# wilkinsdr/raytrace_cpu

Measured on AMD Instinct MI355X. Metric: rays_per_sec, higher is better.
Workload: dtype f64

## Files before the change

raytrace_cpu_amd/csrc/kr_trace.hip:

```cpp

#include <hip/hip_runtime.h>

#include <algorithm>
#include <atomic>
#include <cmath>
#include <cstdio>
#include <cstdlib>
#include <cstring>
#include <iterator>
#include <limits>
#include <map>
#include <mutex>
#include <type_traits>
#include <vector>

#include "kr_common.hpp"
#include "kr_device.hpp"
#include "kr_post_device.hpp"
#include "kr_ray_io.hpp"

namespace kr {

namespace {

constexpr int kBlock = 256;
constexpr int kTraceBlock = 64;
#ifndef KR_REFILL_MIN
#define KR_REFILL_MIN 4
#endif
constexpr int kLongRaySteps = 2048;
#ifndef KR_OCC_STATS
#define KR_OCC_STATS 0
#endif
enum CounterWord { kHead, kTraced, kSteps, kAttempts, kRejects, kStationary, kExtrapolated, kLongest, kCounterWords,
                   kFlagged = kTraced };
constexpr int kCounters = KR_OCC_STATS ? 13 : kCounterWords;
enum CounterBlock { kMainBlock, kSideBlock, kOverflowBlock, kSplitBlock, kCounterBlocks };
constexpr int kListCap = 32768;

template <typename T> struct RayOf;
template <> struct RayOf<double> { using type = kr_ray_f64; };
template <> struct RayOf<float> { using type = kr_ray_f32; };

KR_DEV unsigned long long wave_max(unsigned long long v)
{
#pragma unroll
    for (int off = 32; off > 0; off >>= 1) {
        const unsigned long long o = __shfl_down(v, off, 64);
        v = o > v ? o : v;
    }
    return v;
}

template <typename T> KR_DEV unsigned long long wave_sum(unsigned long long v)
{
#pragma unroll
    for (int off = 32; off > 0; off >>= 1) v += __shfl_down(v, off, 64);
    return v;
}

#define KR_WAVES_ATTR __attribute__((amdgpu_waves_per_eu(HOG ? 1 : METHOD == KR_RK4 ? 3 : METHOD == KR_RK45 ? 2 : 4, 8)))
template <typename T> struct TraceDesc {
    typename RayOf<T>::type* rays;
    long long n;
    TraceConsts<T> c;
    unsigned long long* counters;
    const int* list = nullptr;
    const unsigned long long* n_ptr = nullptr;
    const unsigned char* mask = nullptr;
    int n_mode = 0, mask_want = 0;
};

template <typename T, int METHOD, bool USE_DEST, bool FAST, bool HOG, int REFILL_MIN>
KR_DEV void trace_body(typename RayOf<T>::type* __restrict__ rays, long long n, const TraceConsts<T>& c, unsigned long long* __restrict__ counters,
                       const int* __restrict__ list, const unsigned long long* __restrict__ n_ptr, int n_mode, const unsigned char* __restrict__ mask, int mask_want,
                       int& has_prio, long long first_slot = -1, unsigned long long head_offset = 0)
{
    if (n_ptr) {
        const long long m = (long long) *n_ptr;
        n = (n_mode == 1) ? (m < n ? m : n) : (m > (long long) kListCap ? n : 0);
    }
    const int lane = threadIdx.x & 63;
    const unsigned long long lane_bit = 1ull << lane;

    Lane<T> s;
    long long idx = -1;
    bool have = false;
    bool pend = false;
    bool exhausted = false;
    unsigned long long my_steps = 0, my_traced = 0;
    int32_t my_longest = 0;
    uint32_t my_attempts = 0, my_rejects = 0, my_stationary = 0, my_creep = 0;

#if KR_OCC_STATS
    unsigned long long occ_iters = 0, occ_tail_iters = 0, occ_tail_steps = 0, occ_refills = 0, occ_refill_lanes = 0;
#endif
    for (;;) {
        const unsigned long long need = __builtin_amdgcn_ballot_w64(!have);
        const int n_need = __popcll(need);
        const bool any_have = (need != ~0ull);

        const bool visit = !exhausted && n_need > 0 && (n_need >= REFILL_MIN || !any_have);
        const bool leaving = !visit && !any_have;
        if (visit || leaving) {
            if (pend) {
                my_steps += (unsigned long long) s.steps;
                my_longest = s.steps > my_longest ? s.steps : my_longest;
                store_ray(&rays[idx], s, finish_status<T, USE_DEST>(s, c));
                pend = false;
            }
            if (leaving) break;
            if constexpr (!HOG) {
                const int32_t st = have ? s.steps : 0;
                auto any = [](bool x) { return __builtin_amdgcn_ballot_w64(x) != 0; };
                const int want_prio = any(st > 8 * kLongRaySteps) ? 3 : any(st > 3 * kLongRaySteps) ? 2 : any(st > kLongRaySteps) ? 1 : 0;
                if (want_prio != has_prio) {
                    has_prio = want_prio;
                    switch (want_prio) {
                        case 3: __builtin_amdgcn_s_setprio(3); break;
                        case 2: __builtin_amdgcn_s_setprio(2); break;
                        case 1: __builtin_amdgcn_s_setprio(1); break;
                        default: __builtin_amdgcn_s_setprio(0); break;
                    }
                }
            }
#if KR_OCC_STATS
            ++occ_refills; occ_refill_lanes += n_need;
#endif
            const int leader = __ffsll((long long) need) - 1;
            unsigned long long base = 0;
            if (first_slot >= 0) {
                base = (unsigned long long) first_slot;
                first_slot = -1;
            } else {
                if (lane == leader) base = atomicAdd(&counters[kHead], (unsigned long long) n_need);
                base = __shfl(base, leader, 64) + head_offset;
            }
            if (base + (unsigned long long) n_need >= (unsigned long long) n) exhausted = true;
            if (!have) {
                const long long slot = (long long) base + __popcll(need & (lane_bit - 1));
                if (slot < n) {
                    long long mine = slot;
                    if constexpr (HOG) { if (list) mine = (long long) list[slot]; }
                    const unsigned char* launch = mask ? mask + slot : (const unsigned char*) &rays[mine];
                    const unsigned char launch_of_ray = *launch;
                    load_ray(&rays[mine], s);
                    if ((!mask || launch_of_ray == (unsigned char) mask_want) && s.steps0 >= 0 && s.steps0 < c.steplim) {
                        idx = mine;
                        have = true;
                        ++my_traced;
                        s.steps = 0;
                        s.r_was_positive = false;
                        s.theta_was_positive = true;
                        s.in_retry = false;
                        s.creep_m = 0;
                        s.creep_run = 0;
                        s.creep_mode = false;
                        s.fsal_valid = false;
                        energy_guard_set(s);
                        if (METHOD == KR_RK45) rk45_seed(s, c);
                        if (!loop_cond<T, USE_DEST>(s, c)) {
                            have = false;
                            pend = true;
                        }
                    }
                }
            }
            continue;
        }

        int replay_batch = 1;
        if constexpr (METHOD == KR_RK45 && sizeof(T) == 8) {
            if (!__any(have && !s.creep_mode)) replay_batch = 16;
        }
#if KR_OCC_STATS
        ++occ_iters;
        if (exhausted) { ++occ_tail_iters; occ_tail_steps += have ? 1 : 0; }
#endif
        if (have) {
            bool fin;
            if (METHOD == KR_EULER) fin = step_fixed<T, false, USE_DEST, FAST, HOG>(s, c);
            else if (METHOD == KR_RK4) fin = step_fixed<T, true, USE_DEST, FAST, HOG>(s, c);
            else fin = step_rk45<T, USE_DEST, FAST, HOG>(s, c, my_attempts, my_rejects, my_stationary, my_creep, replay_batch);
            if (fin) {
                have = false;
                pend = true;
            }
        }
    }
    const unsigned long long w_traced = wave_sum<T>(my_traced);
    const unsigned long long w_steps = wave_sum<T>(my_steps);
    const unsigned long long w_att = wave_sum<T>((unsigned long long) my_attempts);
    const unsigned long long w_rej = wave_sum<T>((unsigned long long) my_rejects);
    const unsigned long long w_sta = wave_sum<T>((unsigned long long) my_stationary);
    const unsigned long long w_creep = wave_sum<T>((unsigned long long) my_creep);
    const unsigned long long w_longest = wave_max((unsigned long long) my_longest);
#if KR_OCC_STATS
    {
        const unsigned long long w_tail_steps = wave_sum<T>(occ_tail_steps);
        if (lane == 0) {
            atomicAdd(&counters[8], occ_iters); atomicAdd(&counters[9], occ_tail_iters); atomicAdd(&counters[10], w_tail_steps);
            atomicAdd(&counters[11], occ_refills); atomicAdd(&counters[12], occ_refill_lanes);
        }
    }
#endif
    if (lane == 0) {
        if (w_longest) atomicMax(&counters[kLongest], w_longest);
        if (w_sta) atomicAdd(&counters[kStationary], w_sta);
        if (w_creep) atomicAdd(&counters[kExtrapolated], w_creep);
        if (w_traced) atomicAdd(&counters[kTraced], w_traced);
        if (w_steps) atomicAdd(&counters[kSteps], w_steps);
        if (w_att) atomicAdd(&counters[kAttempts], w_att);
        if (w_rej) atomicAdd(&counters[kRejects], w_rej);
    }
}

template <typename T> KR_DEV void consts_into_vector_registers(TraceConsts<T>& c)
{
    if constexpr (sizeof(T) == 8) {
        auto hold = [](T& x) { asm("" : "+v"(x)); };
        hold(c.a); hold(c.horizon); hold(c.rlim); hold(c.precision); hold(c.theta_precision); hold(c.max_tstep); hold(c.tol);
        hold(c.inv_precision); hold(c.inv_theta_precision); hold(c.tstep_rlim_eff); hold(c.phistep_eff); hold(c.theta_lo); hold(c.theta_hi);
    }
}

template <typename T, int METHOD, bool USE_DEST, bool FAST, bool HOG, int REFILL_MIN>
__global__ void __attribute__((amdgpu_flat_work_group_size(kTraceBlock, kTraceBlock))) KR_WAVES_ATTR
trace_kernel(typename RayOf<T>::type* __restrict__ rays, long long n, TraceConsts<T> c, unsigned long long* __restrict__ counters,
             const int* __restrict__ list, const unsigned long long* __restrict__ n_ptr, int n_mode, const unsigned char* __restrict__ mask, int mask_want)
{
    if (HOG) asm volatile("; claim the whole register file" ::: "v255", "a255");
    int has_prio = 0;
    if constexpr (HOG) {
        if constexpr (METHOD != KR_RK4) consts_into_vector_registers(c);
        trace_body<T, METHOD, USE_DEST, FAST, HOG, REFILL_MIN>(rays, n, c, counters, list, n_ptr, n_mode, mask, mask_want, has_prio, (long long) blockIdx.x * 64,
                                                               (unsigned long long) gridDim.x * 64);
    } else {
        trace_body<T, METHOD, USE_DEST, FAST, HOG, REFILL_MIN>(rays, n, c, counters, list, n_ptr, n_mode, mask, mask_want, has_prio);
    }
}

template <typename T, int METHOD, bool USE_DEST, bool FAST, bool HOG, int REFILL_MIN>
__global__ void __attribute__((amdgpu_flat_work_group_size(kTraceBlock, kTraceBlock))) KR_WAVES_ATTR
trace_multi_kernel(const TraceDesc<T>* __restrict__ descs, int n_desc, const int* __restrict__ wave_trace)
{
    if (HOG) asm volatile("; claim the whole register file" ::: "v255", "a255");
    int has_prio = 0;
    const int ti = wave_trace ? wave_trace[blockIdx.x] : (int) (blockIdx.x % (unsigned) n_desc);
    const TraceDesc<T>* d = &descs[ti];
    if constexpr (HOG) {
        const long long g = (long long) (blockIdx.x / (unsigned) n_desc);
        if constexpr (METHOD != KR_RK4) {
            TraceConsts<T> c = d->c;
            consts_into_vector_registers(c);
            trace_body<T, METHOD, USE_DEST, FAST, HOG, REFILL_MIN>(d->rays, d->n, c, d->counters, d->list, d->n_ptr, d->n_mode, d->mask, d->mask_want, has_prio, g * 64,
                                                                   (unsigned long long) (gridDim.x / (unsigned) n_desc) * 64);
        } else {
            trace_body<T, METHOD, USE_DEST, FAST, HOG, REFILL_MIN>(d->rays, d->n, d->c, d->counters, d->list, d->n_ptr, d->n_mode, d->mask, d->mask_want, has_prio, g * 64,
                                                                   (unsigned long long) (gridDim.x / (unsigned) n_desc) * 64);
        }
    } else {
        trace_body<T, METHOD, USE_DEST, FAST, HOG, REFILL_MIN>(d->rays, d->n, d->c, d->counters, d->list, d->n_ptr, d->n_mode, d->mask, d->mask_want, has_prio);
    }
}

KR_DEV bool ill_conditioned(double k, double h, double Q, double theta, double a)
{
    double sn, cs;
    kr_sincos_f64(theta, sn, cs);
    const double kac = k * a * cs;
    const double hcs = h * cs / sn;
    const double prod = (kac + hcs) * (kac - hcs);
    const double sum = Q + prod;
    return !(__builtin_fabs(sum) > 1e-9 * (__builtin_fabs(Q) + __builtin_fabs(prod))) || !(__builtin_fabs(h) >= 1e-13);
}

KR_DEV unsigned char classify_append(bool strict, long long i, int* __restrict__ list_strict, unsigned long long* __restrict__ n_strict)
{
    const unsigned long long m = __ballot(strict);
    unsigned char mine = 0;
    if (m != 0) {
        const int lane = threadIdx.x & 63;
        const int leader = __ffsll((long long) m) - 1;
        unsigned long long base = 0;
        if (lane == leader) base = atomicAdd(n_strict, (unsigned long long) __popcll(m));
        base = __shfl(base, leader, 64);
        if (strict) {
            const unsigned long long slot = base + __popcll(m & ((1ull << lane) - 1));
            if (slot < (unsigned long long) kListCap) { list_strict[slot] = (int) i; mine = 1; }
            else mine = 2;
        }
    }
    return mine;
}

__global__ void __launch_bounds__(kBlock)
classify_kernel(const kr_ray_f64* __restrict__ rays, long long n, double a, unsigned char* __restrict__ strict_mask, int* __restrict__ list_strict,
                unsigned long long* __restrict__ n_strict)
{
    const long long i = blockIdx.x * (long long) kBlock + threadIdx.x;
    if (i >= n) return;
    const kr_ray_f64* ray = &rays[i];
    bool strict = false;
    if (ray->steps >= 0) strict = ill_conditioned(ray->k, ray->h, ray->Q, ray->theta, a);
    strict_mask[i] = classify_append(strict, i, list_strict, n_strict);
}

struct Workspace {
    int device = 0;
    int cus = 0;
    unsigned long long* counters = nullptr;
    unsigned long long* h_counters = nullptr;
    int* list = nullptr;
    unsigned char* mask = nullptr;
    int64_t mask_capacity = 0;
    std::vector<void*> retired;
    hipStream_t side_stream = nullptr;
    hipEvent_t ev0 = nullptr, ev1 = nullptr;
    hipEvent_t ev_strict0 = nullptr, ev_strict1 = nullptr;
    hipEvent_t ev_main0 = nullptr, ev_main1 = nullptr;
    hipEvent_t ev_classified = nullptr, done = nullptr;
    hipEvent_t ev_in = nullptr;
    void* d_descs = nullptr;
    void* h_descs = nullptr;
    bool leased = false;
    bool pending = false;
    bool split = false;
    int64_t n = 0;
};

unsigned long long* block(const Workspace* ws, CounterBlock which) { return ws->counters + which * kCounters; }
const unsigned long long* host_block(const Workspace* ws, CounterBlock which) { return ws->h_counters + which * kCounters; }
constexpr size_t kCounterBytes = kCounterBlocks * kCounters * sizeof(unsigned long long);

constexpr size_t kMaxPool = 512;
constexpr int kMaxBatch = 256;
constexpr int kMaxMultiGrid = 32768;

constexpr size_t kMaxSideStreams = 16;

constexpr int kMaxDevices = 64;
struct DeviceState {
    std::vector<Workspace*> pool;
    std::map<hipStream_t, hipStream_t> side_streams;
    std::map<hipStream_t, int> side_users;
    hipStream_t poll_stream = nullptr;
    unsigned long long* poll_word = nullptr;
};
std::mutex g_mu, g_poll_mu;
DeviceState g_devices[kMaxDevices];

DeviceState* device_state(int dev)
{
    if (dev < 0 || dev >= kMaxDevices) { set_error("device ordinal out of range"); return nullptr; }
    return &g_devices[dev];
}

int side_stream_for(int dev, hipStream_t user, hipStream_t* out)
{
    DeviceState* ds = device_state(dev);
    if (!ds) return KR_EINVAL;
    std::lock_guard<std::mutex> lk(g_mu);
    auto& table = ds->side_streams;
    auto& users = ds->side_users;
    auto it = table.find(user);
    if (it == table.end()) {
        hipStream_t s = nullptr;
        if (users.size() >= kMaxSideStreams) {
            auto pick = users.begin();
            std::advance(pick, (size_t) (((uintptr_t) user) >> 8) % users.size());
            s = pick->first;
        } else {
            int least = 0, greatest = 0;
            KR_HIP(hipDeviceGetStreamPriorityRange(&least, &greatest));
            KR_HIP(hipStreamCreateWithPriority(&s, hipStreamNonBlocking, least));
        }
        ++users[s];
        it = table.emplace(user, s).first;
    }
    *out = it->second;
    return KR_OK;
}

void workspace_destroy(Workspace* w)
{
    if (!w) return;
    for (void* d : {(void*) w->counters, (void*) w->list, (void*) w->mask, w->d_descs}) if (d) (void) hipFree(d);
    for (void* h : {(void*) w->h_counters, w->h_descs}) if (h) (void) hipHostFree(h);
    for (void* old : w->retired) (void) hipFree(old);
    for (hipEvent_t e : {w->ev0, w->ev1, w->ev_strict0, w->ev_strict1, w->ev_main0, w->ev_main1, w->ev_classified, w->done, w->ev_in})
        if (e) (void) hipEventDestroy(e);
    delete w;
}

int workspace_create(int dev, Workspace** out)
{
    Workspace* w = new Workspace();
    w->device = dev;
    auto fail = [&](int rc) { workspace_destroy(w); return rc; };
#define KR_WS(call) do { hipError_t e__ = (call); if (e__ != hipSuccess) return fail(kr::hip_fail(e__, #call, __FILE__, __LINE__)); } while (0)
    KR_WS(hipMalloc((void**) &w->counters, kCounterBytes));
    KR_WS(hipHostMalloc((void**) &w->h_counters, kCounterBytes, hipHostMallocDefault));
    KR_WS(hipMalloc((void**) &w->list, kListCap * sizeof(int)));
    for (hipEvent_t* timed : {&w->ev0, &w->ev1, &w->ev_strict0, &w->ev_strict1, &w->ev_main0, &w->ev_main1}) KR_WS(hipEventCreate(timed));
    for (hipEvent_t* untimed : {&w->ev_classified, &w->done, &w->ev_in}) KR_WS(hipEventCreateWithFlags(untimed, hipEventDisableTiming));
    hipDeviceProp_t prop;
    KR_WS(hipGetDeviceProperties(&prop, dev));
#undef KR_WS
    w->cus = prop.multiProcessorCount;
    *out = w;
    return KR_OK;
}

int workspace_mask_reserve(Workspace* ws, int64_t n)
{
    if (ws->mask_capacity >= n) return KR_OK;
    const int64_t want = std::max<int64_t>(n, ws->mask_capacity + ws->mask_capacity / 2);
    unsigned char* grown = nullptr;
    KR_HIP(hipMalloc((void**) &grown, (size_t) want));
    if (ws->mask) ws->retired.push_back(ws->mask);
    ws->mask = grown;
    ws->mask_capacity = want;
    return KR_OK;
}

int workspace_acquire(Workspace** out)
{
    int dev = 0;
    KR_HIP(hipGetDevice(&dev));
    DeviceState* ds = device_state(dev);
    if (!ds) return KR_EINVAL;
    Workspace* wait_for = nullptr;
    {
        std::lock_guard<std::mutex> lk(g_mu);
        for (Workspace* w : ds->pool) {
            if (w->leased) continue;
            if (w->pending) {
                if (hipEventQuery(w->done) != hipSuccess) { (void) hipGetLastError(); if (!wait_for) wait_for = w; continue; }
                w->pending = false;
            }
            w->leased = true;
            *out = w;
            return KR_OK;
        }
        if (ds->pool.size() < kMaxPool) {
            Workspace* w = nullptr;
            const int rc = workspace_create(dev, &w);
            if (rc != KR_OK) return rc;
            w->leased = true;
            ds->pool.push_back(w);
            *out = w;
            return KR_OK;
        }
        if (!wait_for) { set_error("kr_trace: too many trace tickets outstanding on this device (kr_trace_wait releases them)"); return KR_EINVAL; }
        wait_for->leased = true;
    }
    KR_HIP(hipEventSynchronize(wait_for->done));
    wait_for->pending = false;
    *out = wait_for;
    return KR_OK;
}

void workspace_release(Workspace* w)
{
    std::lock_guard<std::mutex> lk(g_mu);
    w->leased = false;
}

constexpr int64_t kIsolateMinRays = 1 << 18;

template <typename F>
int with_instance(int integrator, bool dest, F&& f)
{
    using std::integral_constant;
    switch (integrator) {
        case KR_EULER: return f(integral_constant<int, KR_EULER>(), std::false_type());
        case KR_RK4: return dest ? f(integral_constant<int, KR_RK4>(), std::true_type()) : f(integral_constant<int, KR_RK4>(), std::false_type());
        default: return dest ? f(integral_constant<int, KR_RK45>(), std::true_type()) : f(integral_constant<int, KR_RK45>(), std::false_type());
    }
}

struct GridPolicy {
    int max_blocks_per_cu = 0;
    int exact = 0;
    static GridPolicy occupancy(int max_blocks_per_cu) { return GridPolicy{max_blocks_per_cu, 0}; }
    static GridPolicy exactly(int workgroups) { return GridPolicy{0, workgroups}; }
};

template <typename T, int METHOD, bool USE_DEST, bool FAST, bool HOG = false>
int launch(const TraceDesc<T>& d, GridPolicy policy, int cus, hipStream_t stream)
{
    auto kern = trace_kernel<T, METHOD, USE_DEST, FAST, HOG, KR_REFILL_MIN>;
    static std::atomic<int> occ{0};
    int blocks_per_cu = occ.load(std::memory_order_relaxed);
    if (blocks_per_cu == 0) {
        int v = 0;
        KR_HIP(hipOccupancyMaxActiveBlocksPerMultiprocessor(&v, kern, kTraceBlock, 0));
        blocks_per_cu = v < 1 ? 1 : v;
        occ.store(blocks_per_cu, std::memory_order_relaxed);
    }
    int want = policy.max_blocks_per_cu > 0 ? policy.max_blocks_per_cu : (METHOD == KR_EULER && FAST) ? 4 : ((d.n >= 20000000 || (FAST && d.n >= 5000000)) ? 3 : 2);
    if (const char* e = getenv("KR_BLOCKS_PER_CU")) {
        const int v = atoi(e);
        if (v >= 1) want = v;
    }
    want *= 4;
    if (want < blocks_per_cu) blocks_per_cu = want;
    const int64_t resident = (int64_t) cus * blocks_per_cu;
    const int64_t wanted = ((int64_t) d.n + kTraceBlock - 1) / kTraceBlock;
    const int grid = policy.exact > 0 ? policy.exact : (int) std::max<int64_t>(1, std::min(resident, wanted));
    if (!HOG && d.list) { set_error("kr_trace: only side launches work from a list"); return KR_EINVAL; }
    hipLaunchKernelGGL(kern, dim3(grid), dim3(kTraceBlock), 0, stream, d.rays, d.n, d.c, d.counters, d.list, d.n_ptr, d.n_mode, d.mask, d.mask_want);
    KR_HIP(hipGetLastError());
    return KR_OK;
}

template <bool FAST, bool HOG>
int launch_f64(const kr_params* p, const TraceDesc<double>& d, GridPolicy policy, int cus, hipStream_t stream)
{
    return with_instance(p->integrator, p->stop_kind != KR_STOP_THETA, [&](auto method, auto dest) -> int {
        return launch<double, decltype(method)::value, decltype(dest)::value, FAST, HOG>(d, policy, cus, stream);
    });
}

template <bool FAST, bool HOG>
int launch_multi_f64(int integrator, bool dest, const TraceDesc<double>* d_descs, int n_desc, const int* d_wave_trace, int grid, hipStream_t stream)
{
    return with_instance(integrator, dest, [&](auto method, auto use_dest) -> int {
        auto kern = trace_multi_kernel<double, decltype(method)::value, decltype(use_dest)::value, FAST, HOG, KR_REFILL_MIN>;
        hipLaunchKernelGGL(kern, dim3(grid), dim3(kTraceBlock), 0, stream, d_descs, n_desc, d_wave_trace);
        KR_HIP(hipGetLastError());
        return KR_OK;
    });
}

struct SplitPlan {
    TraceDesc<double> side;
    TraceDesc<double> main;
    TraceDesc<double> overflow;
    bool has_overflow = false;
};

int plan_split(const kr_params* p, kr_ray_f64* rays, int64_t n, int steplim, Workspace* ws, SplitPlan* plan)
{
    if (n > 0x7fffffff) { set_error("kr_trace: the split path indexes rays with 32 bits"); return KR_EINVAL; }
    const int rc = workspace_mask_reserve(ws, n);
    if (rc != KR_OK) return rc;
    const unsigned long long* flagged = block(ws, kSplitBlock) + kFlagged;
    const TraceDesc<double> all{rays, (long long) n, make_consts<double>(p, steplim), nullptr};
    plan->side = plan->main = plan->overflow = all;
    plan->side.n = (long long) std::min<int64_t>(n, kListCap);
    plan->side.counters = block(ws, kSideBlock);
    plan->side.list = ws->list;
    plan->side.n_ptr = flagged;
    plan->side.n_mode = 1;
    plan->main.counters = block(ws, kMainBlock);
    plan->main.mask = ws->mask;
    plan->main.mask_want = 0;
    plan->overflow.counters = block(ws, kOverflowBlock);
    plan->overflow.n_ptr = flagged;
    plan->overflow.n_mode = 2;
    plan->overflow.mask = ws->mask;
    plan->overflow.mask_want = 2;
    plan->has_overflow = n > kListCap;
    return KR_OK;
}

int enqueue_classify(const SplitPlan& plan, Workspace* ws, hipStream_t stream)
{
    const long long n = plan.main.n;
    const int cgrid = (int) ((n + kBlock - 1) / kBlock);
    hipLaunchKernelGGL(classify_kernel, dim3(cgrid), dim3(kBlock), 0, stream, plan.main.rays, n, plan.main.c.a, ws->mask, ws->list, block(ws, kSplitBlock) + kFlagged);
    KR_HIP(hipGetLastError());
    return KR_OK;
}

int validate(const kr_params* p, void* d_rays, int64_t n)
{
    if (!p || n < 0 || (n > 0 && !d_rays)) { set_error("kr_trace: null argument or negative n"); return KR_EINVAL; }
    if (p->integrator < KR_EULER || p->integrator > KR_RK45) { set_error("kr_trace: unknown integrator"); return KR_EINVAL; }
    if (p->stop_kind < KR_STOP_THETA || p->stop_kind > KR_STOP_FLATPLANE) { set_error("kr_trace: unknown stop_kind"); return KR_EINVAL; }
    if (p->stop_kind != KR_STOP_THETA && p->integrator == KR_EULER) {
        set_error("kr_trace: Integrator::Euler does not support RayDestination stopping conditions");
        return KR_EINVAL;
    }
    return require_device();
}

int begin_trace(Workspace* ws, hipStream_t stream)
{
    KR_HIP(hipMemsetAsync(ws->counters, 0, kCounterBytes, stream));
    KR_HIP(hipEventRecord(ws->ev0, stream));
    return KR_OK;
}

int end_trace(Workspace* ws, hipStream_t stream)
{
    KR_HIP(hipEventRecord(ws->ev1, stream));
    KR_HIP(hipMemcpyAsync(ws->h_counters, ws->counters, kCounterBytes, hipMemcpyDeviceToHost, stream));
    KR_HIP(hipEventRecord(ws->done, stream));
    return KR_OK;
}

struct Pending {
    const kr_params* p = nullptr;
    void* d_rays = nullptr;
    int64_t n = 0;
    hipStream_t stream = nullptr;
    bool f32 = false, hybrid = false, split = false;
    int steplim = 0;
    Workspace* ws = nullptr;
    SplitPlan plan;
};

int split_front(Pending& t)
{
    Workspace* ws = t.ws;
    int rc = plan_split(t.p, (kr_ray_f64*) t.d_rays, t.n, t.steplim, ws, &t.plan);
    if (rc != KR_OK) return rc;
    rc = enqueue_classify(t.plan, ws, t.stream);
    if (rc != KR_OK) return rc;
    KR_HIP(hipEventRecord(ws->ev_classified, t.stream));
    KR_HIP(hipEventRecord(ws->ev_strict0, t.stream));
    const int grid = (int) std::max<int64_t>(1, std::min<int64_t>((t.plan.side.n + kTraceBlock - 1) / kTraceBlock, (int64_t) (ws->cus / 2) * 4));
    rc = launch_f64<false, true>(t.p, t.plan.side, GridPolicy::exactly(grid), ws->cus, t.stream);
    if (rc != KR_OK) return rc;
    KR_HIP(hipEventRecord(ws->ev_strict1, t.stream));
    ws->split = true;
    return KR_OK;
}

int split_back(Pending& t)
{
    Workspace* ws = t.ws;
    const int mb = KR_FLAG_GET_BLOCKS_PER_CU(t.p->flags);
    KR_HIP(hipStreamWaitEvent(ws->side_stream, ws->ev_classified, 0));
    KR_HIP(hipEventRecord(ws->ev_main0, ws->side_stream));
    const GridPolicy main_waves = GridPolicy::occupancy(mb ? mb : (t.hybrid && t.p->integrator == KR_EULER) ? 4 : 3);
    int rc = t.hybrid ? launch_f64<true, false>(t.p, t.plan.main, main_waves, ws->cus, ws->side_stream)
                      : launch_f64<false, false>(t.p, t.plan.main, main_waves, ws->cus, ws->side_stream);
    if (rc != KR_OK) return rc;
    if (t.plan.has_overflow) {
        rc = launch_f64<false, false>(t.p, t.plan.overflow, GridPolicy::occupancy(mb), ws->cus, ws->side_stream);
        if (rc != KR_OK) return rc;
    }
    KR_HIP(hipEventRecord(ws->ev_main1, ws->side_stream));
    KR_HIP(hipStreamWaitEvent(t.stream, ws->ev_main1, 0));
    return KR_OK;
}

template <typename T>
int dispatch(const Pending& t)
{
    const TraceDesc<T> d{(typename RayOf<T>::type*) t.d_rays, (long long) t.n, make_consts<T>(t.p, t.steplim), block(t.ws, kMainBlock)};
    const GridPolicy policy = GridPolicy::occupancy(KR_FLAG_GET_BLOCKS_PER_CU(t.p->flags));
    return with_instance(t.p->integrator, t.p->stop_kind != KR_STOP_THETA, [&](auto method, auto dest) -> int {
        if constexpr (std::is_same<T, double>::value) {
            if (t.p->flags & KR_FLAG_FAST_MATH) return launch<T, decltype(method)::value, decltype(dest)::value, true>(d, policy, t.ws->cus, t.stream);
        }
        return launch<T, decltype(method)::value, decltype(dest)::value, false>(d, policy, t.ws->cus, t.stream);
    });
}

int trace_front(Pending& t, bool batch)
{
    int rc = validate(t.p, t.d_rays, t.n);
    if (rc != KR_OK) return rc;
    if (t.n == 0) return KR_OK;
    t.steplim = effective_steplim(t.p);
    rc = workspace_acquire(&t.ws);
    if (rc != KR_OK) return rc;
    Workspace* ws = t.ws;
    ws->split = false;
    ws->n = t.n;
    t.hybrid = !t.f32 && (t.p->flags & KR_FLAG_HYBRID) && !(t.p->flags & KR_FLAG_FAST_MATH);
    const bool isolate = !t.f32 && !t.hybrid && !(t.p->flags & KR_FLAG_FAST_MATH) && (t.n >= kIsolateMinRays || (batch && t.n >= 4096)) && !getenv("KR_NO_ISOLATE");
    t.split = t.hybrid || isolate;
    rc = begin_trace(ws, t.stream);
    if (rc != KR_OK || !t.split) return rc;
    rc = side_stream_for(ws->device, t.stream, &ws->side_stream);
    if (rc != KR_OK) return rc;
    return split_front(t);
}

int trace_back(Pending& t)
{
    if (t.n == 0 || !t.ws) return KR_OK;
    const int rc = t.f32 ? dispatch<float>(t) : t.split ? split_back(t) : dispatch<double>(t);
    if (rc != KR_OK) return rc;
    return end_trace(t.ws, t.stream);
}

void abandon(Pending& t)
{
    if (!t.ws) return;
    (void) hipDeviceSynchronize();
    (void) hipGetLastError();
    {
        std::lock_guard<std::mutex> lk(g_mu);
        t.ws->pending = false;
    }
    workspace_release(t.ws);
    t.ws = nullptr;
}

void hand_over(Pending& t, void** ticket)
{
    if (t.ws) {
        std::lock_guard<std::mutex> lk(g_mu);
        t.ws->pending = true;
    }
    *ticket = t.ws;
}

}

int trace_async(const kr_params* p, void* d_rays, int64_t n, hipStream_t stream, bool f32, void** ticket)
{
    *ticket = nullptr;
    Pending t;
    t.p = p; t.d_rays = d_rays; t.n = n; t.stream = stream; t.f32 = f32;
    int rc = trace_front(t, false);
    if (rc == KR_OK) rc = trace_back(t);
    if (rc != KR_OK) { abandon(t); return rc; }
    hand_over(t, ticket);
    return KR_OK;
}

int merged_batch(std::vector<Pending>& ts, bool hybrid)
{
    const int count = (int) ts.size();
    const kr_params* p0 = ts[0].p;
    const bool dest = p0->stop_kind != KR_STOP_THETA;
    hipStream_t primary = ts[0].stream;
    for (auto& t : ts) {
        t.steplim = effective_steplim(t.p);
        int rc = workspace_acquire(&t.ws);
        if (rc != KR_OK) return rc;
        t.ws->split = true;
        t.ws->n = t.n;
    }
    Workspace* w0 = ts[0].ws;
    hipStream_t side = nullptr;
    int rc = side_stream_for(w0->device, primary, &side);
    if (rc != KR_OK) return rc;
    const size_t table_off = 3 * kMaxBatch * sizeof(TraceDesc<double>);
    const size_t staging_bytes = table_off + kMaxMultiGrid * sizeof(int);
    if (!w0->d_descs) {
        KR_HIP(hipMalloc(&w0->d_descs, staging_bytes));
        KR_HIP(hipHostMalloc(&w0->h_descs, staging_bytes, hipHostMallocDefault));
    }
    for (auto& t : ts)
        if (t.stream != primary) {
            KR_HIP(hipEventRecord(t.ws->ev_in, t.stream));
            KR_HIP(hipStreamWaitEvent(primary, t.ws->ev_in, 0));
        }
    TraceDesc<double>* h = (TraceDesc<double>*) w0->h_descs;
    TraceDesc<double>* hog = h, * mainv = h + kMaxBatch, * rest = h + 2 * kMaxBatch;
    int n_rest = 0;
    int64_t hog_max = 1, main_waves = 0, n_total = 0;
    for (int i = 0; i < count; i++) {
        Pending& t = ts[i];
        Workspace* ws = t.ws;
        ws->side_stream = side;
        rc = plan_split(t.p, (kr_ray_f64*) t.d_rays, t.n, t.steplim, ws, &t.plan);
        if (rc == KR_OK) rc = begin_trace(ws, primary);
        if (rc == KR_OK) rc = enqueue_classify(t.plan, ws, primary);
        if (rc != KR_OK) return rc;
        hog[i] = t.plan.side;
        mainv[i] = t.plan.main;
        if (t.plan.has_overflow) rest[n_rest++] = t.plan.overflow;
        hog_max = std::max<int64_t>(hog_max, (t.plan.side.n + kTraceBlock - 1) / kTraceBlock);
        main_waves += (t.n + kTraceBlock - 1) / kTraceBlock;
        n_total += t.n;
    }
    const int mb = KR_FLAG_GET_BLOCKS_PER_CU(p0->flags);
    const int64_t resident = (int64_t) w0->cus * 4 * (mb ? mb : (hybrid && p0->integrator == KR_EULER) ? 4 : 3);
    const int main_grid = (int) std::max<int64_t>(count, std::min<int64_t>({main_waves, 2 * resident, (int64_t) kMaxMultiGrid}));
    int* wave_trace = (int*) ((char*) w0->h_descs + table_off);
    {
        std::vector<std::pair<double, int>> order;
        order.reserve((size_t) main_grid + (size_t) count);
        for (int i = 0; i < count; i++) {
            const int64_t q = std::max<int64_t>(1, (int64_t) ((double) (main_grid - count) * (double) ts[i].n / (double) n_total) + 1);
            for (int64_t k = 0; k < q; k++) order.emplace_back(((double) k + 0.5) / (double) q + 1e-9 * i, i);
        }
        std::sort(order.begin(), order.end());
        for (int b = 0; b < main_grid; b++) wave_trace[b] = order[(size_t) b % order.size()].second;
    }
    KR_HIP(hipMemcpyAsync(w0->d_descs, w0->h_descs, staging_bytes, hipMemcpyHostToDevice, primary));
    const TraceDesc<double>* d = (const TraceDesc<double>*) w0->d_descs;
    const int* d_wave_trace = (const int*) ((const char*) w0->d_descs + table_off);
    KR_HIP(hipEventRecord(w0->ev_classified, primary));
    for (auto& t : ts) KR_HIP(hipEventRecord(t.ws->ev_strict0, primary));
    const int64_t hog_per_trace = std::max<int64_t>(4, std::min<int64_t>(hog_max, (4 * (int64_t) w0->cus) / count));
    rc = launch_multi_f64<false, true>(p0->integrator, dest, d, count, nullptr, (int) (hog_per_trace * count), primary);
    if (rc != KR_OK) return rc;
    for (auto& t : ts) KR_HIP(hipEventRecord(t.ws->ev_strict1, primary));
    KR_HIP(hipStreamWaitEvent(side, w0->ev_classified, 0));
    for (auto& t : ts) KR_HIP(hipEventRecord(t.ws->ev_main0, side));
    rc = hybrid ? launch_multi_f64<true, false>(p0->integrator, dest, d + kMaxBatch, count, d_wave_trace, main_grid, side)
                : launch_multi_f64<false, false>(p0->integrator, dest, d + kMaxBatch, count, d_wave_trace, main_grid, side);
    if (rc != KR_OK) return rc;
    if (n_rest > 0) {
        rc = launch_multi_f64<false, false>(p0->integrator, dest, d + 2 * kMaxBatch, n_rest, nullptr, (int) std::min<int64_t>((int64_t) n_rest * 64, resident), side);
        if (rc != KR_OK) return rc;
    }
    for (auto& t : ts) KR_HIP(hipEventRecord(t.ws->ev_main1, side));
    KR_HIP(hipStreamWaitEvent(primary, ts.back().ws->ev_main1, 0));
    for (auto& t : ts) {
        rc = end_trace(t.ws, primary);
        if (rc != KR_OK) return rc;
        if (t.stream != primary) KR_HIP(hipStreamWaitEvent(t.stream, t.ws->done, 0));
    }
    return KR_OK;
}

int trace_batch_async(int count, const kr_params* const* p, void* const* d_rays, const int64_t* n, void* const* streams, void** tickets)
{
    if (count < 0 || (count > 0 && (!p || !d_rays || !n || !tickets))) { set_error("kr_trace_batch_async: null argument"); return KR_EINVAL; }
    std::vector<Pending> ts((size_t) count);
    for (int i = 0; i < count; i++) {
        tickets[i] = nullptr;
        ts[i].p = p[i]; ts[i].d_rays = d_rays[i]; ts[i].n = n[i]; ts[i].stream = streams ? (hipStream_t) streams[i] : nullptr;
    }
    int rc = KR_OK;
    bool merge = count >= 2 && count <= kMaxBatch && !getenv("KR_NO_MERGED_BATCH") && !getenv("KR_NO_ISOLATE");
    for (int i = 0; i < count && merge; i++) {
        if (validate(p[i], d_rays[i], n[i]) != KR_OK || n[i] < 4096 || (p[i]->flags & KR_FLAG_FAST_MATH)) merge = false;
        else if (p[i]->integrator != p[0]->integrator || (p[i]->stop_kind != KR_STOP_THETA) != (p[0]->stop_kind != KR_STOP_THETA) ||
                 (p[i]->flags & KR_FLAG_HYBRID) != (p[0]->flags & KR_FLAG_HYBRID) || KR_FLAG_GET_BLOCKS_PER_CU(p[i]->flags) != KR_FLAG_GET_BLOCKS_PER_CU(p[0]->flags))
            merge = false;
    }
    if (merge) {
        rc = merged_batch(ts, (p[0]->flags & KR_FLAG_HYBRID) != 0);
    } else {
        for (int i = 0; i < count && rc == KR_OK; i++) rc = trace_front(ts[i], true);
        for (int i = 0; i < count && rc == KR_OK; i++) rc = trace_back(ts[i]);
    }
    if (rc != KR_OK) {
        for (auto& t : ts) abandon(t);
        return rc;
    }
    for (int i = 0; i < count; i++) hand_over(ts[i], &tickets[i]);
    return KR_OK;
}

int trace_wait(void* ticket, kr_stats* stats)
{
    if (stats) std::memset(stats, 0, sizeof(*stats));
    if (!ticket) return KR_OK;
    Workspace* ws = (Workspace*) ticket;
    auto body = [&]() -> int {
        KR_HIP(hipEventSynchronize(ws->done));
        if (!stats) return KR_OK;
        const unsigned long long* mainb = host_block(ws, kMainBlock), * side = host_block(ws, kSideBlock), * over = host_block(ws, kOverflowBlock);
        unsigned long long h[kCounterWords];
        for (int i = 0; i < kCounterWords; i++) h[i] = mainb[i] + side[i] + over[i];
        h[kLongest] = std::max(mainb[kLongest], std::max(side[kLongest], over[kLongest]));
#if KR_OCC_STATS
        for (CounterBlock b : {kMainBlock, kSideBlock, kOverflowBlock}) {
            const unsigned long long* q = host_block(ws, b);
            if (q[8]) std::fprintf(stderr, "kr_occ: launch %d (0 main, 1 strict side, 2 overflow): steps %llu wave_iters %llu step-loop lane occupancy %.4f | after queue exhaustion: "
                                   "wave_iters %llu (%.2f %%) lane occupancy %.4f | refills %llu lanes/refill %.2f | longest ray %llu steps\n", (int) b, q[kSteps], q[8], (double) q[kSteps] / (64.0 * q[8]), q[9],
                                   100.0 * q[9] / q[8], q[9] ? (double) q[10] / (64.0 * q[9]) : 0.0, q[11], q[11] ? (double) q[12] / q[11] : 0.0, q[kLongest]);
        }
#endif
        stats->rays_total = ws->n;
        stats->rays_strict_side = (int64_t) host_block(ws, kSplitBlock)[kFlagged];
        stats->rays_traced = (int64_t) h[kTraced];
        stats->steps_total = (int64_t) h[kSteps];
        stats->rk45_attempts = (int64_t) h[kAttempts];
        stats->rk45_rejects = (int64_t) h[kRejects];
        stats->rk45_stationary_steps = (int64_t) h[kStationary];
        stats->rk45_extrapolated_steps = (int64_t) h[kExtrapolated];
        stats->longest_ray_steps = (int64_t) h[kLongest];
        stats->longest_ray_steps_strict_side = ws->split ? (int64_t) side[kLongest] : 0;
        stats->steps_strict_side = ws->split ? (int64_t) side[kSteps] : 0;
        stats->rk45_evaluated_strict_side = ws->split ? (int64_t) (side[kAttempts] - side[kStationary] - side[kExtrapolated]) : 0;
        float ms = 0;
        KR_HIP(hipEventElapsedTime(&ms, ws->ev0, ws->ev1));
        stats->kernel_ms = ms;
        if (ws->split) {
            KR_HIP(hipEventElapsedTime(&ms, ws->ev_strict0, ws->ev_strict1));
            stats->strict_side_ms = ms;
            KR_HIP(hipEventElapsedTime(&ms, ws->ev_main0, ws->ev_main1));
            stats->main_ms = ms;
        }
        return KR_OK;
    };
    const int rc = body();
    {
        std::lock_guard<std::mutex> lk(g_mu);
        if (rc == KR_OK) ws->pending = false;
        ws->leased = false;
    }
    return rc;
}

int trace_poll(void* ticket, int64_t* rays_started, int32_t* finished)
{
    if (rays_started) *rays_started = 0;
    if (finished) *finished = 1;
    if (!ticket) return KR_OK;
    Workspace* ws = (Workspace*) ticket;
    const hipError_t q = hipEventQuery(ws->done);
    if (q == hipSuccess) {
        if (rays_started) *rays_started = ws->n;
        return KR_OK;
    }
    (void) hipGetLastError();
    if (q != hipErrorNotReady) return kr::hip_fail(q, "hipEventQuery(trace)", __FILE__, __LINE__);
    if (finished) *finished = 0;
    int dev = 0;
    KR_HIP(hipGetDevice(&dev));
    if (dev != ws->device) { set_error("kr_trace_poll: the ticket belongs to another device than the current one"); return KR_EINVAL; }
    DeviceState* ds = device_state(dev);
    if (!ds) return KR_EINVAL;
    std::lock_guard<std::mutex> lk(g_poll_mu);
    if (!ds->poll_stream) {
        KR_HIP(hipStreamCreateWithFlags(&ds->poll_stream, hipStreamNonBlocking));
        KR_HIP(hipHostMalloc((void**) &ds->poll_word, sizeof(unsigned long long), hipHostMallocDefault));
    }
    KR_HIP(hipMemcpyAsync(ds->poll_word, block(ws, kMainBlock) + kHead, sizeof(unsigned long long), hipMemcpyDeviceToHost, ds->poll_stream));
    KR_HIP(hipStreamSynchronize(ds->poll_stream));
    if (rays_started) *rays_started = (int64_t) std::min<unsigned long long>(*ds->poll_word, (unsigned long long) ws->n);
    return KR_OK;
}

void trace_release(void* ticket)
{
    if (ticket) workspace_release((Workspace*) ticket);
}

void side_stream_forget(hipStream_t user)
{
    hipStream_t side = nullptr;
    int side_dev = -1;
    {
        std::lock_guard<std::mutex> lk(g_mu);
        for (int dev = 0; dev < kMaxDevices && side_dev < 0; dev++) {
            DeviceState& ds = g_devices[dev];
            auto it = ds.side_streams.find(user);
            if (it == ds.side_streams.end()) continue;
            hipStream_t s = it->second;
            ds.side_streams.erase(it);
            auto u = ds.side_users.find(s);
            if (u != ds.side_users.end() && --u->second <= 0) {
                ds.side_users.erase(u);
                side = s;
                side_dev = dev;
            } else {
                return;
            }
        }
    }
    if (!side) return;
    CurrentDeviceGuard restore;
    if (hipSetDevice(side_dev) == hipSuccess) {
        (void) hipStreamSynchronize(side);
        (void) hipStreamDestroy(side);
    }
}

int trace_shutdown()
{
    CurrentDeviceGuard restore;
    std::lock_guard<std::mutex> lk(g_mu);
    for (const DeviceState& ds : g_devices)
        for (const Workspace* w : ds.pool)
            if (w->leased) {
                set_error("kr_shutdown: trace tickets are outstanding (kr_trace_wait / kr_trace_release them first)");
                return KR_EINVAL;
            }
    for (int dev = 0; dev < kMaxDevices; dev++) {
        DeviceState& ds = g_devices[dev];
        if (ds.pool.empty() && ds.side_users.empty() && !ds.poll_stream) continue;
        if (hipSetDevice(dev) != hipSuccess) { (void) hipGetLastError(); continue; }
        (void) hipDeviceSynchronize();
        for (Workspace* w : ds.pool) workspace_destroy(w);
        ds.pool.clear();
        {
            std::lock_guard<std::mutex> pl(g_poll_mu);
            if (ds.poll_stream) { (void) hipStreamDestroy(ds.poll_stream); ds.poll_stream = nullptr; }
            if (ds.poll_word) { (void) hipHostFree(ds.poll_word); ds.poll_word = nullptr; }
        }
        for (auto& kv : ds.side_users) (void) hipStreamDestroy(kv.first);
        ds.side_users.clear();
        ds.side_streams.clear();
    }
    return KR_OK;
}

int trace_dev(const kr_params* p, void* d_rays, int64_t n, hipStream_t stream, kr_stats* stats, bool f32)
{
    if (stats) { std::memset(stats, 0, sizeof(*stats)); stats->rays_total = n; }
    void* ticket = nullptr;
    const int rc = trace_async(p, d_rays, n, stream, f32, &ticket);
    if (rc != KR_OK) return rc;
    if (!stats) { trace_release(ticket); return KR_OK; }
    const int rc2 = trace_wait(ticket, stats);
    stats->rays_total = n;
    return rc2;
}

}
```

Measured before the change: 154.6 million.

## Claim ray runs in 64-ray blocks per wave and prefetch upcoming rays

In the non-hog path, each wave now claims a private run of kRunBlock rays from the global head counter, not exactly as many as it needs. Later refills draw from that run without an atomic. The last ~10% of rays (or at least two blocks per workgroup) are handed out dynamically so the tail stays balanced. After each refill the wave touches the cache lines of the next few rays in its run so their loads are warm. This cuts head-atomic traffic and ray-load latency, at the cost of coarser work distribution and extra speculative loads.

```diff
diff --git a/raytrace_cpu_amd/csrc/kr_trace.hip b/raytrace_cpu_amd/csrc/kr_trace.hip
--- a/raytrace_cpu_amd/csrc/kr_trace.hip
+++ b/raytrace_cpu_amd/csrc/kr_trace.hip
@@ -28,13 +28,26 @@
 #ifndef KR_REFILL_MIN
 #define KR_REFILL_MIN 4
 #endif
+#ifndef KR_RUN_BLOCK
+#define KR_RUN_BLOCK 64
+#endif
+#ifndef KR_RUN_DYN_1024
+#define KR_RUN_DYN_1024 102
+#endif
+#ifndef KR_RUN_PREFETCH
+#define KR_RUN_PREFETCH 8
+#endif
+constexpr int kRunBlock = KR_RUN_BLOCK;
+constexpr int kRunDynamicShare = KR_RUN_DYN_1024;
+constexpr int kRunDynamicBlocks = 2;
+constexpr int kRunPrefetch = KR_RUN_PREFETCH;
 constexpr int kLongRaySteps = 2048;
 #ifndef KR_OCC_STATS
 #define KR_OCC_STATS 0
 #endif
 enum CounterWord { kHead, kTraced, kSteps, kAttempts, kRejects, kStationary, kExtrapolated, kLongest, kCounterWords,
                    kFlagged = kTraced };
-constexpr int kCounters = KR_OCC_STATS ? 13 : kCounterWords;
+constexpr int kCounters = KR_OCC_STATS ? 17 : kCounterWords;
 enum CounterBlock { kMainBlock, kSideBlock, kOverflowBlock, kSplitBlock, kCounterBlocks };
 constexpr int kListCap = 32768;
 
@@ -91,9 +104,42 @@
     unsigned long long my_steps = 0, my_traced = 0;
     int32_t my_longest = 0;
     uint32_t my_attempts = 0, my_rejects = 0, my_stationary = 0, my_creep = 0;
+    long long run_cur = 0, run_limit = 0;
+    int run_left = 0;
+    bool run_blocks = false, head_passed = false;
+    uint32_t touched = 0;
+    if constexpr (!HOG && kRunBlock > 0) {
+        const long long per_visit = (n * kRunDynamicShare) >> 10, least = (long long) kRunDynamicBlocks * kRunBlock * (long long) gridDim.x;
+        const long long dyn = per_visit > least ? per_visit : least;
+        run_limit = n > dyn ? n - dyn : 0;
+        run_blocks = run_limit > 0;
+    }
+
+    auto start_ray = [&](long long mine, unsigned char launch_of_ray) {
+        if ((!mask || launch_of_ray == (unsigned char) mask_want) && s.steps0 >= 0 && s.steps0 < c.steplim) {
+            idx = mine;
+            have = true;
+            ++my_traced;
+            s.steps = 0;
+            s.r_was_positive = false;
+            s.theta_was_positive = true;
+            s.in_retry = false;
+            s.creep_m = 0;
+            s.creep_run = 0;
+            s.creep_mode = false;
+            s.fsal_valid = false;
+            energy_guard_set(s);
+            if (METHOD == KR_RK45) rk45_seed(s, c);
+            if (!loop_cond<T, USE_DEST>(s, c)) {
+                have = false;
+                pend = true;
+            }
+        }
+    };
 
 #if KR_OCC_STATS
     unsigned long long occ_iters = 0, occ_tail_iters = 0, occ_tail_steps = 0, occ_refills = 0, occ_refill_lanes = 0;
+    unsigned long long occ_store_wait = 0, occ_claim_wait = 0, occ_record_wait = 0, occ_claims = 0;
 #endif
     for (;;) {
         const unsigned long long need = __builtin_amdgcn_ballot_w64(!have);
@@ -103,6 +149,10 @@
         const bool visit = !exhausted && n_need > 0 && (n_need >= REFILL_MIN || !any_have);
         const bool leaving = !visit && !any_have;
         if (visit || leaving) {
+            if constexpr (!HOG && kRunPrefetch > 0) asm volatile("" :: "v"(touched));
+#if KR_OCC_STATS
+            const unsigned long long occ_t0 = __builtin_amdgcn_s_memtime();
+#endif
             if (pend) {
                 my_steps += (unsigned long long) s.steps;
                 my_longest = s.steps > my_longest ? s.steps : my_longest;
@@ -128,43 +178,106 @@
             ++occ_refills; occ_refill_lanes += n_need;
 #endif
             const int leader = __ffsll((long long) need) - 1;
-            unsigned long long base = 0;
-            if (first_slot >= 0) {
-                base = (unsigned long long) first_slot;
-                first_slot = -1;
-            } else {
-                if (lane == leader) base = atomicAdd(&counters[kHead], (unsigned long long) n_need);
-                base = __shfl(base, leader, 64) + head_offset;
-            }
-            if (base + (unsigned long long) n_need >= (unsigned long long) n) exhausted = true;
-            if (!have) {
-                const long long slot = (long long) base + __popcll(need & (lane_bit - 1));
-                if (slot < n) {
-                    long long mine = slot;
-                    if constexpr (HOG) { if (list) mine = (long long) list[slot]; }
-                    const unsigned char* launch = mask ? mask + slot : (const unsigned char*) &rays[mine];
-                    const unsigned char launch_of_ray = *launch;
-                    load_ray(&rays[mine], s);
-                    if ((!mask || launch_of_ray == (unsigned char) mask_want) && s.steps0 >= 0 && s.steps0 < c.steplim) {
-                        idx = mine;
-                        have = true;
-                        ++my_traced;
-                        s.steps = 0;
-                        s.r_was_positive = false;
-                        s.theta_was_positive = true;
-                        s.in_retry = false;
-                        s.creep_m = 0;
-                        s.creep_run = 0;
-                        s.creep_mode = false;
-                        s.fsal_valid = false;
-                        energy_guard_set(s);
-                        if (METHOD == KR_RK45) rk45_seed(s, c);
-                        if (!loop_cond<T, USE_DEST>(s, c)) {
-                            have = false;
-                            pend = true;
+            if constexpr (HOG) {
+                unsigned long long base = 0;
+                if (first_slot >= 0) {
+                    base = (unsigned long long) first_slot;
+                    first_slot = -1;
+                } else {
+                    if (lane == leader) base = atomicAdd(&counters[kHead], (unsigned long long) n_need);
+                    base = __shfl(base, leader, 64) + head_offset;
+                }
+                if (base + (unsigned long long) n_need >= (unsigned long long) n) exhausted = true;
+                if (!have) {
+                    const long long slot = (long long) base + __popcll(need & (lane_bit - 1));
+                    if (slot < n) {
+                        long long mine = slot;
+                        if (list) mine = (long long) list[slot];
+                        const unsigned char* launch = mask ? mask + slot : (const unsigned char*) &rays[mine];
+                        const unsigned char launch_of_ray = *launch;
+                        load_ray(&rays[mine], s);
+                        if ((!mask || launch_of_ray == (unsigned char) mask_want) && s.steps0 >= 0 && s.steps0 < c.steplim) {
+                            idx = mine;
+                            have = true;
+                            ++my_traced;
+                            s.steps = 0;
+                            s.r_was_positive = false;
+                            s.theta_was_positive = true;
+                            s.in_retry = false;
+                            s.creep_m = 0;
+                            s.creep_run = 0;
+                            s.creep_mode = false;
+                            s.fsal_valid = false;
+                            energy_guard_set(s);
+                            if (METHOD == KR_RK45) rk45_seed(s, c);
+                            if (!loop_cond<T, USE_DEST>(s, c)) {
+                                have = false;
+                                pend = true;
+                            }
                         }
                     }
                 }
+            } else {
+#if KR_OCC_STATS
+                __builtin_amdgcn_s_waitcnt(0x0F70);
+                const unsigned long long occ_t1 = __builtin_amdgcn_s_memtime();
+#endif
+                const int rank = __popcll(need & (lane_bit - 1));
+                const int take = run_left < n_need ? run_left : n_need;
+                long long slot = run_cur + rank;
+                if (take < n_need) {
+                    const int rest = n_need - take;
+                    const int ask = (run_blocks && rest < kRunBlock) ? kRunBlock : rest;
+                    unsigned long long fresh = 0;
+                    if (lane == leader) fresh = atomicAdd(&counters[kHead], (unsigned long long) ask);
+                    fresh = __shfl(fresh, leader, 64);
+                    if (rank >= take) slot = (long long) fresh + (rank - take);
+                    run_cur = (long long) fresh + rest;
+                    run_left = ask - rest;
+                    if ((long long) fresh >= run_limit) run_blocks = false;
+                    if ((long long) fresh + ask >= n) {
+                        head_passed = true;
+                        const long long room = n - run_cur;
+                        run_left = room <= 0 ? 0 : room < (long long) run_left ? (int) room : run_left;
+                    }
+#if KR_OCC_STATS
+                    ++occ_claims;
+#endif
+                } else {
+                    run_cur += n_need;
+                    run_left -= n_need;
+                }
+                exhausted = head_passed && run_left == 0;
+#if KR_OCC_STATS
+                asm volatile("" :: "v"(slot));
+                const unsigned long long occ_t2 = __builtin_amdgcn_s_memtime();
+                unsigned long long occ_t3 = occ_t2;
+#endif
+                const bool entering = !have && slot < n;
+                unsigned char launch_of_ray = 0;
+                if (entering) {
+                    const unsigned char* launch = mask ? mask + slot : (const unsigned char*) &rays[slot];
+                    launch_of_ray = *launch;
+                    load_ray(&rays[slot], s);
+#if KR_OCC_STATS
+                    asm volatile("" :: "v"(s.eq_cross));
+                    occ_t3 = __builtin_amdgcn_s_memtime();
+#endif
+                    start_ray(slot, launch_of_ray);
+                }
+                if constexpr (kRunPrefetch > 0) {
+                    const int ahead = run_left < kRunPrefetch ? run_left : kRunPrefetch;
+                    const int bytes = ahead * (int) sizeof(typename RayOf<T>::type), off = lane * 128;
+                    const unsigned char* line = nullptr;
+                    if (ahead > 0) {
+                        if (off < bytes + 128) line = (const unsigned char*) &rays[run_cur] + (off < bytes ? off : bytes - 1);
+                        else if (mask && lane == 63) line = mask + run_cur;
+                    }
+                    if (line) touched = *line;
+                }
+#if KR_OCC_STATS
+                occ_store_wait += occ_t1 - occ_t0; occ_claim_wait += occ_t2 - occ_t1; occ_record_wait += occ_t3 - occ_t2;
+#endif
             }
             continue;
         }
@@ -201,6 +314,7 @@
         if (lane == 0) {
             atomicAdd(&counters[8], occ_iters); atomicAdd(&counters[9], occ_tail_iters); atomicAdd(&counters[10], w_tail_steps);
             atomicAdd(&counters[11], occ_refills); atomicAdd(&counters[12], occ_refill_lanes);
+            atomicAdd(&counters[13], occ_store_wait); atomicAdd(&counters[14], occ_claim_wait); atomicAdd(&counters[15], occ_record_wait); atomicAdd(&counters[16], occ_claims);
         }
     }
 #endif
@@ -864,6 +978,8 @@
             if (q[8]) std::fprintf(stderr, "kr_occ: launch %d (0 main, 1 strict side, 2 overflow): steps %llu wave_iters %llu step-loop lane occupancy %.4f | after queue exhaustion: "
                                    "wave_iters %llu (%.2f %%) lane occupancy %.4f | refills %llu lanes/refill %.2f | longest ray %llu steps\n", (int) b, q[kSteps], q[8], (double) q[kSteps] / (64.0 * q[8]), q[9],
                                    100.0 * q[9] / q[8], q[9] ? (double) q[10] / (64.0 * q[9]) : 0.0, q[11], q[11] ? (double) q[12] / q[11] : 0.0, q[kLongest]);
+            if (q[11] && b != kSideBlock) std::fprintf(stderr, "kr_occ: launch %d visits %llu head atomics %llu | cycles per visit: store wait %.1f claim %.1f record wait %.1f\n", (int) b, q[11], q[16],
+                                                      (double) q[13] / q[11], (double) q[14] / q[11], (double) q[15] / q[11]);
         }
 #endif
         stats->rays_total = ws->n;
```

Result: no change. 153.2 million (-0.9%).
